# przemektmalon/SeqALib

Hardware: AMD Instinct MI355X
Metric: GCUPS (DP cell updates/s) on batched 4k×4k SW; bit-exact score match (higher is better)
Workload: dtype f16 (integer-exact below 2048); 1 GPU; sw_batch_10000x4096x4096; pairs_per_gpu=10000, total_pairs=10000, m=4096, n=4096, algo=SmithWatermanSA, match=equal<char>, parallelism=pair-shard x1

## Files before the change

### seqalib_amd/csrc/sa_api.hip

```cpp
#include <hip/hip_runtime.h>
#include <limits.h>
#include <sched.h>
#include <stdio.h>
#include <stdlib.h>
#include <string.h>

#include <algorithm>
#include <atomic>
#include <functional>
#include <condition_variable>
#include <memory>
#include <mutex>
#include <chrono>
#include <string>
#include <thread>
#include <vector>

#include "sa_dc.h"
#include "sa_internal.h"

using namespace sa;

namespace sa {
bool dna2_pack(uint8_t* dst, const uint8_t* src, uint64_t n);
// ... 459 lines not shown
        if (algo != SA_SW && algo != SA_NW && algo != SA_LOCAL_GOTOH && algo != SA_GLOBAL_GOTOH) return T16Mode{};
        const int64_t mi = is_affine(algo) ? 2 * ((int64_t)sc0->gap_open + sc0->gap_extend) - 1 : 2 * (int64_t)sc0->gap - 1;
        if (mi < INT_MIN / 4) return T16Mode{};
        eff.mismatch = (int32_t)mi;
        eff.allow_mismatch = 1;
    }
    const sa_scoring* sc = &eff;
    T16Mode t;
    t.mismatch = sc->mismatch;
    if (algo == SA_LOCAL_GOTOH || algo == SA_GLOBAL_GOTOH) return t16_mode_affine(algo, sc, max_m, max_n);
    if (algo != SA_SW && algo != SA_NW) return t;
    const int64_t MA = sc->match, MI = sc->mismatch, G = sc->gap;
    if (MA < -32 || MA > 31 || MI < -32 || MI > 31) return t;
    if (G > 0 || MI > MA || G < -4096) return t;
    if (algo == SA_SW && G == 0) return t;
    if (max_n >= 65535) return t;
    const int64_t m = max_m, n = max_n, k = std::min(m, n);
    if (algo == SA_SW) {
        t.ok = true;
        if (4 * std::max<int64_t>(MA, 0) * k + 3 > 32767) t.retry_above = (int32_t)(8191 - std::max<int64_t>(MA, 0));
        return t;
    }
    auto hi_at = [&](int64_t i, int64_t j) {
        return std::max(std::min(i, j) * MA + (i > j ? i - j : j - i) * G, (i + j) * G);
    };
    auto lo_at = [&](int64_t i, int64_t j) {
        return std::max(std::min(i, j) * MI + (i > j ? i - j : j - i) * G, (i + j) * G);
    };
    int64_t hi = INT64_MIN, lo = INT64_MAX;
    const int64_t pts[7][2] = {{0, 0}, {m, 0}, {0, n}, {k, k}, {m, n}, {k, n}, {m, k}};
    for (auto& q : pts) {
        hi = std::max(hi, hi_at(q[0], q[1]));
        lo = std::min(lo, lo_at(q[0], q[1]));
    }
    const int64_t cand_lo = lo + std::min<int64_t>(std::min(MI, G), 0);
    const int64_t delta = (hi + cand_lo) >> 1;
    if (4 * (hi - delta) + 3 > 32767 || 4 * (cand_lo - delta) < -32768) return t;
    t.ok = true;
    t.delta = (int32_t)delta;
    return t;
}

int validate_scoring(sa_ctx* c, int algo, const sa_scoring* s) {
    if (!s) return fail(c, SA_ERR_ARG, "scoring is NULL");
    if (algo < SA_SW || algo > SA_MYERS_MILLER) return fail(c, SA_ERR_ARG, "unknown algorithm");
    return SA_OK;
}

bool f16_hi_exact(int s) {
    if (s < -2048 || s > 2048) return false;
    const _Float16 h = (_Float16)(float)s;
    return (int)(float)h == s && (__builtin_bit_cast(uint16_t, h) & 0xffu) == 0;
}
bool so2_f16_scoring(const sa_ctx* c, int algo, const sa_scoring* sc, const T16Mode& tm) {
    if (algo != SA_SW || !tm.ok || c->f16_off) return false;
    if (const char* e = getenv("SEQALIB_SO2_F16")) if (e[0] == '0') return false;
    return f16_hi_exact(sc->match) && f16_hi_exact(tm.mismatch) && f16_hi_exact(-128);
}

T16Mode t16_candidate(int algo, const sa_scoring* sc, uint32_t max_m, uint32_t max_n, uint32_t npairs) {
    T16Mode t = t16_mode(algo, sc, max_m, max_n);
    if ((algo == SA_SW || algo == SA_LOCAL_GOTOH) && !keyed_ok(algo, sc, max_m, max_n)) t.ok = false;
    if (t.ok && algo == SA_GLOBAL_GOTOH && t.retry_above != INT_MAX &&
        make_variant(algo, max_m, max_n, npairs, true, true).pl.split)
        t.ok = false;
    if (const char* e16 = getenv("SEQALIB_T16")) if (e16[0] == '0') t.ok = false;
    return t;
}

int build_variants(int algo, uint32_t max_m, uint32_t max_n, uint32_t npairs, bool t16, Variant (&vars)[3],
                   bool* has_fb, int only = 0) {
    int nv = 0;
    if (t16 && only != 2) vars[nv++] = make_variant(algo, max_m, max_n, npairs, true, true);
    if (!t16 || only != 1) vars[nv++] = make_variant(algo, max_m, max_n, npairs, false, true);
    *has_fb = false;
    for (int k = 0; k < nv; ++k) *has_fb = *has_fb || vars[k].pl.split;
    if (*has_fb) vars[nv] = make_variant(algo, max_m, max_n, npairs, false, false);
    const int all = nv + (*has_fb ? 1 : 0);
    uint64_t dir_stride = 0;
    for (int k = 0; k < all; ++k) dir_stride = std::max(dir_stride, vars[k].pl.g.dir_slot);
    for (int k = 0; k < all; ++k) {
        vars[k].slot_bytes += dir_stride - vars[k].pl.g.dir_slot;
        vars[k].pl.g.dir_slot = dir_stride;
    }
    return nv;
}

struct HostAlphabet {
    int sel = -1;
    uint32_t prof[5] = {0, 0, 0, 0, 0};
};
HostAlphabet host_alphabet(const uint8_t* s1, uint64_t t1, const uint8_t* s2, uint64_t t2, const uint8_t* lut,
                           int match, int mismatch, bool affine) {
    HostAlphabet h;
    bool seen[256] = {};
    for (uint64_t k = 0; k < t1; ++k) seen[s1[k]] = true;
    for (uint64_t k = 0; k < t2; ++k) seen[s2[k]] = true;
    uint32_t syms[4] = {0, 0, 0, 0};
    int nsym = 0;
    for (int b = 0; b < 256; ++b)
        if (seen[b]) {
            if (nsym == 4) { h.sel = 0; return h; }
            syms[nsym++] = (uint32_t)b;
        }
    for (int b = 0; nsym < 4 && b < 256; ++b)
        if (!seen[b]) syms[nsym++] = (uint32_t)b;
    for (int c = 0; c < 4; ++c) {
        uint32_t w = 0;
        for (int c2 = 0; c2 < 4; ++c2) {
            const bool v = lut ? lut[syms[c] * 256 + syms[c2]] != 0 : syms[c] == syms[c2];
// ... 32 lines not shown
    const bool allow = sc->allow_mismatch != 0;
    const bool bits = d_mbits != nullptr;
    const bool lut = !bits && d_lutbits != nullptr;
    const T16Mode tm = bits ? T16Mode{} : t16_candidate(algo, sc, max_m, max_n, npairs);
    const bool t16 = tm.ok;
    const bool kernel_timing = getenv("SEQALIB_KERNEL_TIMING") != nullptr;
    if (!c->aux) SA_HIP(c, hipMalloc(&c->aux, kPipeSlots * kAuxWords * 4));
    if (!c->h_sel) {
        SA_HIP(c, hipHostMalloc(reinterpret_cast<void**>(&c->h_sel), 64, hipHostMallocDefault));
        SA_HIP(c, hipEventCreateWithFlags(&c->ev_sel, hipEventDisableTiming));
    }
    if (!pipe && c->s_fill) {
        SA_HIP(c, hipStreamSynchronize(c->s_fill));
        SA_HIP(c, hipStreamSynchronize(c->s_tb));
    }
    constexpr int nslots = kPipeSlots;
    const int slot = pipe ? (int)(c->pipe_k % (uint64_t)nslots) : 0;
    uint32_t* aux = c->aux + kAuxWords * slot;
    if (pipe && c->ev_slot[slot]) SA_HIP(c, hipStreamWaitEvent(stream, c->ev_slot[slot], 0));
    if (!c->h_f16) {
        SA_HIP(c, hipHostMalloc(reinterpret_cast<void**>(&c->h_f16), 8, hipHostMallocCoherent));
        *c->h_f16 = 0;
        void* dp = nullptr;
        SA_HIP(c, hipHostGetDevicePointer(&dp, c->h_f16, 0));
        c->d_f16 = static_cast<unsigned long long*>(dp);
    }
    {
        const unsigned long long w = __atomic_load_n(c->h_f16, __ATOMIC_ACQUIRE);
        const uint32_t s = (uint32_t)(w >> 32);
        if (s != 0 && s != c->f16_seen) {
            c->f16_seen = s;
            if (c->f16_seq - s < 4 && (uint64_t)(uint32_t)w * 64 > c->f16_cnt[s & 3]) c->f16_off = true;
        }
    }
    const uint32_t* sel = nullptr;
    const uint32_t* prof = aux + kAuxProf;
    static_assert(kAuxSel == kAuxProf + 5, "profile and selection word: one upload");
    int only = 0;
    HostAlphabet hal;
    if (t16 && hs) hal = host_alphabet(hs->s1, hs->t1, hs->s2, hs->t2, hs->lut, sc->match, tm.mismatch, is_affine(algo));
    const HostAlphabet* ha = &hal;
    const bool host_sel = t16 && ha->sel >= 0;
    if (host_sel) {
        c->host_sel = ha->sel;
        const bool in_hdr = hs->hhdr != nullptr;
        if (!in_hdr && !hs->hprof) return fail(c, SA_ERR_ARG, "internal: no pinned profile slot");
        uint32_t* const hp = in_hdr ? hs->hhdr : hs->hprof;
        for (int k = 0; k < 5; ++k) hp[k] = ha->prof[k];
        hp[5] = (uint32_t)ha->sel;
        if (in_hdr) prof = hs->dhdr;
        else SA_HIP(c, hipMemcpyAsync(aux + kAuxProf, hp, 24, hipMemcpyHostToDevice, stream));
        const Variant vt = make_variant(algo, max_m, max_n, npairs, true, true);
        const bool bu_hand = vt.so && !is_affine(algo) && (vt.pl.g.bands > 1 || vt.segs > 1);
        const bool f16 = vt.so2 && so2_f16_scoring(c, algo, sc, tm);
        if (ha->sel == 0) only = 2;
        else if (tm.retry_above == INT_MAX && !bu_hand && !f16) only = 1;
        else sel = prof + 5;
    }
    if (hs && hs->up_bytes)
        SA_HIP(c, hipMemcpyAsync(hs->up_dst, hs->up_src, hs->up_bytes, hipMemcpyHostToDevice, stream));
    if (host_sel) {
        SA_HIP(c, hipEventRecord(c->ev_sel, stream));
    } else if (t16) {
        c->host_sel = -1;
        SA_HIP(c, launch_alphabet_scan(d1, o1, d2, o2, npairs, aux, stream));
        SA_HIP(c, launch_decide_t16(d_lutbits, sc->match, tm.mismatch, is_affine(algo) ? 1 : 0, aux, stream));
        SA_HIP(c, hipMemcpyAsync(c->h_sel, aux + kAuxSel, 4, hipMemcpyDeviceToHost, stream));
        SA_HIP(c, hipEventRecord(c->ev_sel, stream));
        sel = aux + kAuxSel;
    }
    Variant vars[3];
    bool has_fb = false;
    const int nv = build_variants(algo, max_m, max_n, npairs, t16, vars, &has_fb, only);
    if (const char* e = getenv("SEQALIB_SPLIT_FALLBACK")) has_fb = has_fb && e[0] != '0';
    c->nvar = nv;
    uint64_t slot_bytes = 0, sp_bands = 0;
    bool any_split = false;
    for (int k = 0; k < nv + (has_fb ? 1 : 0); ++k) {
        if (k < nv) {
            c->var_kernel[k] = vars[k].kernel;
            c->var_R[k] = vars[k].pl.R;
            c->var_W[k] = vars[k].pl.split ? 0 : vars[k].pl.W;
            c->var_records[k] = vars[k].so ? SA_RECORDS_SCORE_ONLY : vars[k].t16 ? SA_RECORDS_TAGS : SA_RECORDS_FLAGS;
        }
        slot_bytes = std::max(slot_bytes, vars[k].slot_bytes);
        if (vars[k].pl.split) {
            any_split = true;
            sp_bands = std::max<uint64_t>(sp_bands, vars[k].pl.g.bands);
        }
    }
    const uint64_t budget = pipe ? ws_budget(c) / nslots : ws_budget(c);
    uint64_t per_launch = slot_bytes ? std::max<uint64_t>(1, budget / std::max<uint64_t>(slot_bytes, 1)) : npairs;
    per_launch = std::min<uint64_t>(per_launch, npairs ? npairs : 1);
    per_launch = std::min<uint64_t>(per_launch, 1u << 30);
    const uint64_t need = (per_launch * slot_bytes + 4096 + 255) & ~(uint64_t)255;
    if (need > budget && per_launch == 1 && c->ws_limit)
        return fail(c, SA_ERR_NOMEM, "one pair needs " + std::to_string(slot_bytes) +
                                         " bytes of workspace, above the limit");
    int rc = ensure_ws(c, std::max<uint64_t>(pipe ? nslots * need : need, 4096));
    if (rc) return rc;
    auto al256 = [](uint64_t x) { return (x + 255) & ~(uint64_t)255; };
    uint64_t hand_rb = 0, hand_part = 0, hand_seg = 0;
    for (int k = 0; k < nv; ++k)
        if (vars[k].so && !is_affine(algo)) {
            hand_rb = std::max(hand_rb, al256(per_launch * vars[k].pl.rowbuf_elems * 4));
            hand_part = std::max(hand_part, al256(per_launch * vars[k].part_slot * 8));
            hand_seg = std::max(hand_seg, al256(per_launch * vars[k].seg_slot * 4));
// ... 85 lines not shown
            fp.mbits = d_mbits; fp.mbits_off = d_mbits_off;
            fp.dirs = wbase; fp.dir_slot = pl.g.dir_slot; fp.band_stride = pl.g.band_stride;
            fp.rowbuf = rowbuf; fp.rowbuf_slot = pl.rowbuf_elems;
            fp.res = d_res;
            fp.pair_base = (uint32_t)base;
            fp.max_m = max_m; fp.max_n = max_n;
            fp.gap = sc->gap; fp.match = sc->match;
            fp.mismatch = v.t16 ? tm.mismatch : allow ? sc->mismatch : INT_MIN;
            fp.gap_open = sc->gap_open; fp.gap_extend = sc->gap_extend;
            fp.waves = pl.W;
            fp.count = cnt;
            fp.stage_seq2 = (max_n <= kMaxStagedSeq2 && !no_stage) ? 1 : 0;
            fp.prof = prof;
            const bool fb = k == nv;
            fp.sel = fb ? nullptr : sel; fp.sel_want = v.t16 ? 1u : 0u;
            fp.redo = (!fb && nv == 2 && !v.t16) ? 1 : 0;
            fp.rerun = fb ? 1 : 0;
            fp.t16_delta = v.t16 ? tm.delta : 0;
            fp.retry_above = v.t16 ? tm.retry_above : INT_MAX;
            fp.t16_sent = v.t16 ? tm.sent : -10000;
            fp.snap_h = snap_h; fp.snap_p = snap_p; fp.snap_m = snap_p + per_launch * v.snap_p_slot;
            if (v.so) {
                fp.part_bands = (uint32_t)v.pl.g.bands;
                fp.snap_c = reinterpret_cast<int32_t*>(snap_p + 2 * per_launch * v.snap_p_slot);
                fp.seg_slot = v.seg_slot;
            }
            if (v.so && !is_affine(algo)) {
                fp.epoch = c->hand_tag;
#ifndef SA_R5_CONTROL
                fp.rowbuf = reinterpret_cast<int32_t*>(c->hand);
                fp.band_part = reinterpret_cast<unsigned long long*>(c->hand + hand_rb);
                fp.seg_hand = reinterpret_cast<uint32_t*>(c->hand + hand_rb + hand_part);
#else
                const uintptr_t bp = (reinterpret_cast<uintptr_t>(fp.snap_c + per_launch * v.snap_c_slot) + 7) & ~(uintptr_t)7;
                fp.band_part = reinterpret_cast<unsigned long long*>(bp);
                fp.seg_hand = reinterpret_cast<uint32_t*>(fp.band_part + per_launch * v.part_slot);
#endif
                fp.wait_polls = so_wait_polls;
            }
            fp.snap_h_slot = v.snap_h_slot; fp.snap_p_slot = v.snap_p_slot; fp.snap_nch = v.snap_nch;
            fp.split_bands = (uint32_t)sp_bands;
            fp.ticket = pl.split ? reinterpret_cast<uint32_t*>(vblk) : v.so ? aux + kAuxTicket : nullptr;
            fp.hand = pl.split ? reinterpret_cast<unsigned long long*>(vblk + 256) : nullptr;
            fp.hand_x_off = pl.split ? hand_x_off : 0;
            fp.part = pl.split ? reinterpret_cast<int32_t*>(spbase + sp_part) : nullptr;
            fp.wait_ticks = wait_ticks;
            fp.part_segs = std::max<uint32_t>(1, v.segs);
            if (v.so2) {
                const uint32_t nch = chunks_per_band(max_n);
                const uint32_t sg = std::max(1u, std::min(fp.part_segs, nch / 2));
                const uint32_t range = std::max((nch + sg - 1) / sg, 3u) * kChunk + kWave;
                const uint32_t cap = (range + 15) & ~15u;
                fp.so2_stage = (2 * cap <= 8192 && !no_stage) ? cap : 0;
                if (v.t16 && so2_f16_scoring(c, algo, sc, tm)) {
                    fp.so2_f16 = 1;
                    fp.retry_above = std::min(fp.retry_above, kSo2F16RetryAbove);
                }
            }
            FillVariant fv{pl.R, lut, allow || v.t16, keyed, v.t16, v.cmax, pl.split, bits};
            fv.so = v.so;
            fv.so2 = v.so2;
            return fv;
        };
        const bool tb_on_fill = pipe && nv == 2 && !vars[1].t16 && !vars[1].pl.split;
        auto make_tp = [&](int k) {
            const Variant& v = vars[k];
            TbParams tp{};
            tp.seq1 = d1; tp.off1 = o1; tp.seq2 = d2; tp.off2 = o2;
            tp.lutbits = lut ? d_lutbits : nullptr;
            tp.vrec = bits ? 1 : 0;
            tp.dirs = fps[k].dirs; tp.dir_slot = v.pl.g.dir_slot;
            tp.ops = d_ops; tp.res = d_res;
            tp.pair_base = (uint32_t)base; tp.count = cnt;
            tp.max_m = max_m; tp.max_n = max_n;
            tp.gap = fps[k].gap; tp.match = fps[k].match; tp.mismatch = fps[k].mismatch;
            tp.gap_open = fps[k].gap_open; tp.gap_extend = fps[k].gap_extend;
            tp.allow = (allow || v.t16) ? 1 : 0;
            tp.tagged = v.t16 ? 1 : 0;
            tp.sel = fps[k].sel; tp.sel_want = fps[k].sel_want;
            tp.rerun = fps[k].rerun;
            tp.band_stride = v.pl.g.band_stride;
            tp.snap_h = fps[k].snap_h; tp.snap_p = fps[k].snap_p;
            tp.snap_h_slot = v.snap_h_slot; tp.snap_p_slot = v.snap_p_slot; tp.snap_nch = v.snap_nch;
            tp.prof = fps[k].prof;
            tp.t16_delta = fps[k].t16_delta;
            tp.t16_sent = fps[k].t16_sent;
            tp.so_lp = pipe ? 4 : 8;
            tp.keep_redo = tb_on_fill && k == 1 ? 1 : 0;
            tp.clear_redo = tb_on_fill && k == 0 ? 1 : 0;
#ifdef SA_R5_CONTROL
            tp.keep_redo = tp.clear_redo = 0;
#endif
            return tp;
        };
        for (int k = 0; k < nv; ++k) {
            const Variant& v = vars[k];
            const Plan& pl = v.pl;
            if (v.so && !is_affine(algo))
                if (int rc = next_hand_tag(c, hand_need, sf)) return rc;
            const FillVariant fv = make_fp(k);
            const FillParams& fp = fps[k];
            if (pl.split) SA_HIP(c, hipMemsetAsync(fp.ticket, 0, 256 + hand_x_off * 8 * aff2, sf));
            if (v.so && !is_affine(algo)) SA_HIP(c, hipMemsetAsync(fp.ticket, 0, 8, sf));
            static_assert(kAuxF16Flags == kAuxTicket + 1, "ticket and f16 count: one memset");
            if (kev) SA_HIP(c, hipEventRecord(kev[2 * k], sf));
            const bool units = v.so && !is_affine(algo);
            const uint32_t grid = pl.split ? (uint32_t)(cnt * sp_bands)
                                : units ? (v.so2 ? (cnt + 1) / 2 : cnt) * pl.g.bands * v.segs : cnt;
// ... 1086 lines not shown
```

### seqalib_amd/csrc/sa_fill_so2.hip

```cpp
#include "sa_fill_impl.h"

namespace sa {

namespace {

__device__ __forceinline__ uint32_t pk_max_u16(uint32_t a, uint32_t b) {
    uint32_t d;
    asm("v_pk_max_u16 %0, %1, %2" : "=v"(d) : "v"(a), "v"(b));
    return d;
}
__device__ __forceinline__ uint32_t lo16(uint32_t x) { return x & 0xffffu; }
__device__ __forceinline__ uint32_t lane_here() {
    uint32_t l;
    asm volatile("v_mov_b32 %0, %1" : "=v"(l) : "v"((uint32_t)threadIdx.x));
    return l;
}
__device__ __forceinline__ uint32_t hi16(uint32_t x) { return x >> 16; }
__device__ __forceinline__ uint32_t wave_pk_max(uint32_t v) {
    v = pk_max_u16(v, (uint32_t)__builtin_amdgcn_update_dpp(0, (int)v, 0x111, 0xf, 0xf, false));
    v = pk_max_u16(v, (uint32_t)__builtin_amdgcn_update_dpp(0, (int)v, 0x112, 0xf, 0xf, false));
    v = pk_max_u16(v, (uint32_t)__builtin_amdgcn_update_dpp(0, (int)v, 0x114, 0xf, 0xf, false));
    v = pk_max_u16(v, (uint32_t)__builtin_amdgcn_update_dpp(0, (int)v, 0x118, 0xf, 0xf, false));
    v = pk_max_u16(v, (uint32_t)__builtin_amdgcn_update_dpp(0, (int)v, 0x142, 0xa, 0xf, false));
    v = pk_max_u16(v, (uint32_t)__builtin_amdgcn_update_dpp(0, (int)v, 0x143, 0xc, 0xf, false));
    return v;
}
__device__ __forceinline__ uint32_t pk_max_i16(uint32_t a, uint32_t b) {
    uint32_t d;
    asm("v_pk_max_i16 %0, %1, %2" : "=v"(d) : "v"(a), "v"(b));
    return d;
}
__device__ __forceinline__ uint32_t f16x2_to_u16x2(uint32_t x) {
    uint32_t d;
    asm("v_cvt_u16_f16_sdwa %0, %1 dst_sel:WORD_0 dst_unused:UNUSED_PAD src0_sel:WORD_0\n\t"
        "v_cvt_u16_f16_sdwa %0, %1 dst_sel:WORD_1 dst_unused:UNUSED_PRESERVE src0_sel:WORD_1"
        : "=&v"(d) : "v"(x));
    return d;
}
__device__ __forceinline__ uint32_t u16x2_to_f16x2(uint32_t x) {
    uint32_t d;
    asm("v_cvt_f16_u16_sdwa %0, %1 dst_sel:WORD_0 dst_unused:UNUSED_PAD src0_sel:WORD_0\n\t"
        "v_cvt_f16_u16_sdwa %0, %1 dst_sel:WORD_1 dst_unused:UNUSED_PRESERVE src0_sel:WORD_1"
        : "=&v"(d) : "v"(x));
    return d;
}
__device__ __forceinline__ uint32_t f16_bits(int s) {
    const _Float16 h = (_Float16)(float)s;
    return (uint32_t)__builtin_bit_cast(uint16_t, h);
}

}

template <int ALG, int R, bool FK>
__global__ __launch_bounds__(64) __attribute__((amdgpu_waves_per_eu(4, 4))) void fill_so2_kernel(FillParams P) {
    constexpr bool NWK = ALG == SA_NW;
    static_assert(!(FK && NWK), "the f16 cell is SW's");
    if (sa_skip(P.sel, P.sel_want)) return;
    static_assert(R >= 8 && R % 2 == 0, "the sampled chunk maximum needs 8 rows per lane");
    constexpr int BAND = kWave * R;
    constexpr int SPP = 8;
    extern __shared__ __attribute__((aligned(16))) uint32_t smem[];
    uint32_t* const s_step = smem;
    const int lane = threadIdx.x;
    uint32_t* const s_park = s_step + (lane == 63 ? 96 : 160);
    const uint32_t SEGS = P.part_segs;
    const uint32_t ncp = (P.count + 1) / 2;
    uint32_t t = 0;
    if (lane == 0) t = atomicAdd(P.ticket, 1u);
    t = __builtin_amdgcn_readlane(t, 0);
    const uint32_t rowt = ncp * SEGS;
    const uint32_t band0 = t / rowt;
    const uint32_t rem = t - band0 * rowt;
    const uint32_t seg = rem / ncp;
    const uint32_t cp = rem - seg * ncp;
    const uint32_t sA = 2 * cp;
    const bool hasB = 2 * cp + 1 < P.count;
    const uint32_t sB = hasB ? 2 * cp + 1 : sA;
    const uint32_t pA = P.pair_base + sA, pB = P.pair_base + sB;
    const uint64_t o1A = P.off1[pA], o2A = P.off2[pA], o1B = P.off1[pB], o2B = P.off2[pB];
    const int mA = (int)(P.off1[pA + 1] - o1A), nA = (int)(P.off2[pA + 1] - o2A);
    const int mB = hasB ? (int)(P.off1[pB + 1] - o1B) : 0, nB = hasB ? (int)(P.off2[pB + 1] - o2B) : 0;
    const bool badA = (uint32_t)mA > P.max_m || (uint32_t)nA > P.max_n;
    const bool badB = hasB && ((uint32_t)mB > P.max_m || (uint32_t)nB > P.max_n);
    const int BA = (!badA && mA > 0 && nA > 0) ? (mA + BAND - 1) / BAND : 0;
    const int BB = (hasB && !badB && mB > 0 && nB > 0) ? (mB + BAND - 1) / BAND : 0;
    const int B2 = max(BA, BB);
    const int n2 = max(BA ? nA : 0, BB ? nB : 0);
    if ((int)band0 >= (B2 > 0 ? B2 : 1)) return;
    const uint32_t nch2 = chunks_per_band((uint32_t)n2);
    const uint32_t segs_p = max(1u, min(SEGS, nch2 / 2));
    const uint32_t cps = (nch2 + segs_p - 1) / segs_p;
    const uint32_t c0 = seg * cps, c1 = B2 > 0 ? min(nch2, c0 + cps) : 0u;
    const uint32_t last_seg = (nch2 - 1) / cps;
    if (seg > (B2 > 0 ? last_seg : 0u)) return;
    const uint32_t nchA = chunks_per_band((uint32_t)nA), nchB = chunks_per_band((uint32_t)nB);
    const bool liveA = (int)band0 < BA, liveB = (int)band0 < BB;
    const uint32_t epoch16 = P.epoch << 16;
    const uint32_t symp = P.prof[4];
    const int G = P.gap;
    const int D0 = P.t16_delta;
    auto border2 = [&](int i) __attribute__((always_inline)) -> uint32_t {
        return NWK ? ((uint32_t)(i * G - D0) & 0xffffu) * 0x10001u : 0u;
    };
    uint32_t seg_lost = 0;

    uint32_t cw[4];
#pragma unroll
    for (int c = 0; c < 4; ++c) {
        uint32_t w = 0;
#pragma unroll
        for (int x = 0; x < 4; ++x) {
            const int s = (int)(int8_t)(so_profile(P.prof[x]) >> (8 * c));
            if constexpr (FK) w |= (f16_bits(s) >> 8) << (8 * x);
            else w |= ((uint32_t)(s + 128) & 255u) << (8 * x);
        }
        cw[c] = w;
    }
    const uint8_t* const s1A = P.seq1 + o1A;
    const uint8_t* const s1B = P.seq1 + o1B;
    const uint8_t* const s2A = P.seq2 + o2A;
    const uint8_t* const s2B = P.seq2 + o2B;
    const bool staged = P.so2_stage != 0;
    const int k0 = max(0, (int)(c0 * kChunk) - kWave);
    uint8_t* const s_cA = reinterpret_cast<uint8_t*>(smem + kStepBufWords);
    uint8_t* const s_cB = s_cA + P.so2_stage;
    if (staged) {
        const int k1 = min(n2, (int)(c1 * kChunk));
        for (int k = k0 + lane; k < k1; k += kWave) {
            s_cA[k - k0] = (uint8_t)(liveA && k < nA ? t16_code8(symp, s2A[(uint32_t)k]) >> 3 : 0u);
            s_cB[k - k0] = (uint8_t)(liveB && k < nB ? t16_code8(symp, s2B[(uint32_t)k]) >> 3 : 0u);
        }
        __syncthreads();
    }
    constexpr uint32_t kOut = FK ? 0xd8d8d8d8u : 0u;
    auto col_pair = [&](int c, uint32_t& wa, uint32_t& wb) {
        const bool ia = liveA && c >= 0 && c < nA, ib = liveB && c >= 0 && c < nB;
        uint32_t xa, xb;
        if (staged) {
            xa = ia ? (uint32_t)s_cA[c - k0] : 0u;
            xb = ib ? (uint32_t)s_cB[c - k0] : 0u;
        } else {
            xa = ia ? (t16_code8(symp, s2A[(uint32_t)c]) >> 3) : 0u;
            xb = ib ? (t16_code8(symp, s2B[(uint32_t)c]) >> 3) : 0u;
        }
        wa = ia ? (xa == 0 ? cw[0] : xa == 1 ? cw[1] : xa == 2 ? cw[2] : cw[3]) : kOut;
        wb = ib ? (xb == 0 ? cw[0] : xb == 1 ? cw[1] : xb == 2 ? cw[2] : cw[3]) : kOut;
    };
    const uint32_t G128 = FK ? f16_bits(G) * 0x10001u : ((uint32_t)(G + 128) & 0xffffu) * 0x10001u;
    const uint32_t C128 = 0x00800080u;

    typedef uint32_t __attribute__((address_space(1))) gu32;
    gu32* const rbA = (gu32*)(P.rowbuf + (uint64_t)sA * P.rowbuf_slot);
    gu32* const rbB = (gu32*)(P.rowbuf + (uint64_t)sB * P.rowbuf_slot);
    const uint64_t rbs = P.max_n;

    const int row0 = (int)band0 * BAND + lane * R;
    uint32_t Hp[R], sel[R];
    uint32_t prev_up = border2(row0), colA = 0, colB = 0, cml = 0, smax = 0;
#pragma unroll
    for (int r = 0; r < R; ++r) Hp[r] = border2(row0 + r + 1);
    int capSA = -1, capSB = -1, capIA = 0, capIB = 0;
    uint32_t capA = 0, capB = 0;
    bool tookA = false, tookB = false;
    if constexpr (NWK) {
        if (liveA && mA > 0 && nA > 0 && (int)band0 == (mA - 1) / BAND) {
            capIA = (mA - 1) % BAND;
            capSA = nA - 1 + capIA / R;
        }
        if (liveB && mB > 0 && nB > 0 && (int)band0 == (mB - 1) / BAND) {
            capIB = (mB - 1) % BAND;
            capSB = nB - 1 + capIB / R;
        }
    }
    if (c0 > 0) {
        const uint64_t hoff = ((uint64_t)band0 * SEGS + seg - 1) * (R + 1) * kWave;
        const uint32_t* const hsA = P.seg_hand + (uint64_t)sA * P.seg_slot + hoff;
        const uint32_t* const hsB = P.seg_hand + (uint64_t)sB * P.seg_slot + hoff;
        uint32_t pa_ = 0, pb_ = 0;
        auto rd = [&]() __attribute__((always_inline)) {
#pragma unroll
            for (int r = 0; r < R; ++r) {
                Hp[r] = liveA ? __hip_atomic_load(hsA + (uint32_t)(r * kWave + lane), __ATOMIC_RELAXED, __HIP_MEMORY_SCOPE_AGENT) : epoch16;
                sel[r] = liveB ? __hip_atomic_load(hsB + (uint32_t)(r * kWave + lane), __ATOMIC_RELAXED, __HIP_MEMORY_SCOPE_AGENT) : epoch16;
            }
            pa_ = liveA ? __hip_atomic_load(hsA + (uint32_t)(R * kWave + lane), __ATOMIC_RELAXED, __HIP_MEMORY_SCOPE_AGENT) : epoch16;
            pb_ = liveB ? __hip_atomic_load(hsB + (uint32_t)(R * kWave + lane), __ATOMIC_RELAXED, __HIP_MEMORY_SCOPE_AGENT) : epoch16;
        };
        auto stale = [&]() __attribute__((always_inline)) -> bool {
            bool st = ((pa_ & 0xffff0000u) != epoch16) | ((pb_ & 0xffff0000u) != epoch16);
#pragma unroll
            for (int r = 0; r < R; ++r) st |= ((Hp[r] & 0xffff0000u) != epoch16) | ((sel[r] & 0xffff0000u) != epoch16);
            return st;
        };
        rd();
        for (uint32_t it = 0; !seg_lost && __builtin_amdgcn_ballot_w64(stale()) != 0; ++it) {
            if (it >= P.wait_polls) { seg_lost = 1; break; }
            __builtin_amdgcn_s_sleep(2);
            rd();
        }
#pragma unroll
        for (int r = 0; r < R; ++r) Hp[r] = lo16(Hp[r]) | sel[r] << 16;
        prev_up = lo16(pa_) | pb_ << 16;
        col_pair((int)(c0 * kChunk) - 1 - lane, colA, colB);
    }
#pragma unroll
    for (int r = 0; r < R; ++r) {
        const int row = row0 + r;
        const uint32_t ca = (liveA && row < mA) ? (t16_code8(symp, s1A[(uint32_t)row]) >> 3) : 12u;
        const uint32_t cb = (liveB && row < mB) ? (4u + (t16_code8(symp, s1B[(uint32_t)row]) >> 3)) : 12u;
        sel[r] = FK ? 0x0cu | ca << 8 | 0x0c0000u | cb << 24 : ca | 0x0c00u | cb << 16 | 0x0c000000u;
    }

    auto step = [&](auto ramp, auto gc, int kC, int q0, const uint32_t* sq, const uint32_t* sc, uint32_t* sp,
                    uint32_t& recA, uint32_t& recB) {
        constexpr bool RAMP = decltype(ramp)::value;
        constexpr int g = decltype(gc)::value;
        constexpr int PH = g & 3;
        const int q = q0 + g;
        const uint32_t vh = sq[g];
        const uint32_t va = sc[2 * g], vb = sc[2 * g + 1];
        const uint32_t up = (uint32_t)shr1((int)vh, (int)Hp[R - 1]);
        colA = (uint32_t)shr1((int)va, (int)colA);
        colB = (uint32_t)shr1((int)vb, (int)colB);
        if (!RAMP || kC + q - lane >= 0) {
            uint32_t dcur, pt;
            if constexpr (FK)
                asm("v_perm_b32 %1, %2, %3, %4\n\tv_pk_add_f16 %0, %5, %1"
                    : "=&v"(dcur), "=&v"(pt) : "v"(colB), "v"(colA), "v"(sel[0]), "v"(prev_up));
            else
                asm("v_perm_b32 %1, %2, %3, %4\n\tv_pk_add_u16 %0, %5, %1"
                    : "=&v"(dcur), "=&v"(pt) : "v"(colB), "v"(colA), "v"(sel[0]), "v"(prev_up));
            uint32_t hu = up;
#define SO2_CELL_N(LAST)                                                                          \
    asm("v_perm_b32 %[dn], %[cb], %[ca], %[sn]\n\t"                                                \
        "v_pk_add_u16 %[dn], %[hp], %[dn]\n\t"                                                     \
        "v_pk_max_i16 %[t1], %[hu], %[hp]\n\t"                                                     \
        "v_pk_add_u16 %[t1], %[t1], %[g]\n\t"                                                      \
        "v_pk_max_i16 %[t1], %[t1], %[dr]\n\t" LAST                                                \
        : [t1] "=&v"(t1), [dn] "=&v"(dn), [hp] "+v"(Hp[r])                                         \
        : [dr] "v"(dcur), [hu] "v"(hu), [g] "s"(G128), [c] "s"(C128),                              \
          [sn] "v"(sel[r + 1 < R ? r + 1 : r]), [ca] "v"(colA), [cb] "v"(colB))
#define SO2_CELL_L(LAST)                                                                          \
    asm("v_pk_max_i16 %[t1], %[hu], %[hp]\n\t"                                                     \
        "v_pk_add_u16 %[t1], %[t1], %[g]\n\t"                                                      \
        "v_pk_max_i16 %[t1], %[t1], %[dr]\n\t" LAST                                                \
        : [t1] "=&v"(t1), [hp] "+v"(Hp[r])                                                         \
        : [dr] "v"(dcur), [hu] "v"(hu), [g] "s"(G128), [c] "s"(C128))
#define SO2_CELL_FN                                                                               \
    asm("v_perm_b32 %[dn], %[cb], %[ca], %[sn]\n\t"                                                \
        "v_pk_add_f16 %[dn], %[hp], %[dn]\n\t"                                                     \
        "v_pk_max_i16 %[t1], %[hu], %[hp]\n\t"                                                     \
        "v_pk_add_f16 %[t1], %[t1], %[g]\n\t"                                                      \
        "v_pk_maximum3_f16 %[hp], %[t1], %[dr], 0"                                                 \
        : [t1] "=&v"(t1), [dn] "=&v"(dn), [hp] "+v"(Hp[r])                                         \
        : [dr] "v"(dcur), [hu] "v"(hu), [g] "s"(G128),                                             \
          [sn] "v"(sel[r + 1 < R ? r + 1 : r]), [ca] "v"(colA), [cb] "v"(colB))
#define SO2_CELL_FL                                                                               \
    asm("v_pk_max_i16 %[t1], %[hu], %[hp]\n\t"                                                     \
        "v_pk_add_f16 %[t1], %[t1], %[g]\n\t"                                                      \
        "v_pk_maximum3_f16 %[hp], %[t1], %[dr], 0"                                                 \
        : [t1] "=&v"(t1), [hp] "+v"(Hp[r])                                                         \
        : [dr] "v"(dcur), [hu] "v"(hu), [g] "s"(G128))
#pragma unroll
            for (int r = 0; r < R; ++r) {
                uint32_t t1;
                if (r + 1 < R) {
                    uint32_t dn;
                    if constexpr (FK) SO2_CELL_FN;
                    else if constexpr (NWK) SO2_CELL_N("v_pk_sub_u16 %[hp], %[t1], %[c]");
                    else SO2_CELL_N("v_pk_sub_u16 %[hp], %[t1], %[c] clamp");
                    dcur = dn;
                } else {
                    if constexpr (FK) SO2_CELL_FL;
                    else if constexpr (NWK) SO2_CELL_L("v_pk_sub_u16 %[hp], %[t1], %[c]");
                    else SO2_CELL_L("v_pk_sub_u16 %[hp], %[t1], %[c] clamp");
                }
                if (!NWK && PH == 3 && (r & 7) == 7) {
                    if constexpr (FK) {
                        cml = pk_max_i16(cml, Hp[r - 4]);
                        cml = pk_max_i16(cml, Hp[r]);
                    } else {
                        cml = pk_max_u16(cml, Hp[r - 4]);
                        cml = pk_max_u16(cml, Hp[r]);
                    }
                }
                hu = Hp[r];
            }
#undef SO2_CELL_N
#undef SO2_CELL_L
#undef SO2_CELL_FN
#undef SO2_CELL_FL
            prev_up = up;
        }
        if constexpr (NWK) {
            if (kC + q == capSA) {
                uint32_t v = 0;
#pragma unroll
                for (int r = 0; r < R; ++r) v = r == capIA % R ? Hp[r] : v;
                capA = lane == capIA / R ? lo16(v) : capA;
                tookA = true;
            }
            if (kC + q == capSB) {
                uint32_t v = 0;
#pragma unroll
                for (int r = 0; r < R; ++r) v = r == capIB % R ? Hp[r] : v;
                capB = lane == capIB / R ? hi16(v) : capB;
                tookB = true;
            }
        }
        recA = __builtin_amdgcn_alignbit(Hp[R - 1], recA, 16u);
        recB = __builtin_amdgcn_perm(Hp[R - 1], recB, 0x07060302u);
        sp[g] = Hp[R - 1];
    };

    uint8_t* const dA = P.dirs + (uint64_t)sA * P.dir_slot + (uint64_t)band0 * P.band_stride;
    uint8_t* const dB = P.dirs + (uint64_t)sB * P.dir_slot + (uint64_t)band0 * P.band_stride;
    gu32* const gA = rbA + (uint64_t)(band0 > 0 ? band0 - 1 : 0) * rbs;
    gu32* const gB = rbB + (uint64_t)(band0 > 0 ? band0 - 1 : 0) * rbs;
    gu32* const oA = rbA + (uint64_t)band0 * rbs;
    gu32* const oB = rbB + (uint64_t)band0 * rbs;
    for (uint32_t chunk = c0; chunk < c1; ++chunk) {
        const int kC = (int)chunk * kChunk;
        {
            const uint32_t ln = lane_here();
            const int c = kC + (int)ln;
            const bool in = lane < kChunk;
            uint32_t wa = 0, wb = 0;
            if (in) col_pair(c, wa, wb);
            const bool wantA = in && band0 > 0 && liveA && c < nA, wantB = in && band0 > 0 && liveB && c < nB;
            gu32* const ga = gA + (uint32_t)c;
            gu32* const gb = gB + (uint32_t)c;
            uint32_t ha = lo16(border2(c + 1)), hb = ha;
            if (wantA) ha = __hip_atomic_load(ga, __ATOMIC_RELAXED, __HIP_MEMORY_SCOPE_AGENT);
            if (wantB) hb = __hip_atomic_load(gb, __ATOMIC_RELAXED, __HIP_MEMORY_SCOPE_AGENT);
            if (band0 > 0) {
                for (uint32_t it = 0; !seg_lost; ++it) {
                    const bool st = (wantA && (ha & 0xffff0000u) != epoch16) || (wantB && (hb & 0xffff0000u) != epoch16);
                    if (__builtin_amdgcn_ballot_w64(st) == 0) break;
                    if (it >= P.wait_polls) { seg_lost = 1; break; }
                    __builtin_amdgcn_s_sleep(2);
                    if (wantA) ha = __hip_atomic_load(ga, __ATOMIC_RELAXED, __HIP_MEMORY_SCOPE_AGENT);
                    if (wantB) hb = __hip_atomic_load(gb, __ATOMIC_RELAXED, __HIP_MEMORY_SCOPE_AGENT);
                }
            }
            if (in) {
                s_step[ln] = FK ? u16x2_to_f16x2(lo16(ha) | hb << 16) : lo16(ha) | hb << 16;
                s_step[32 + 2 * ln] = wa;
                s_step[33 + 2 * ln] = wb;
            }
        }
        __syncthreads();
        auto packet = [&](auto rmp, int q0) __attribute__((always_inline)) {
            uint32_t pa[SPP / 2] = {0, 0, 0, 0}, pb[SPP / 2] = {0, 0, 0, 0};
            const uint32_t* const sq = s_step + q0;
            const uint32_t* const sc = s_step + 32 + 2 * q0;
            uint32_t* const sp = s_park + q0;
            auto st = [&](auto gc) __attribute__((always_inline)) {
                constexpr int g = decltype(gc)::value;
                step(rmp, gc, kC, q0, sq, sc, sp, pa[g / 2], pb[g / 2]);
            };
            st(std::integral_constant<int, 0>{});
            st(std::integral_constant<int, 1>{});
            st(std::integral_constant<int, 2>{});
            st(std::integral_constant<int, 3>{});
            st(std::integral_constant<int, 4>{});
            st(std::integral_constant<int, 5>{});
            st(std::integral_constant<int, 6>{});
            st(std::integral_constant<int, 7>{});
            const uint32_t po = ((uint32_t)((kC + q0) / SPP) * kWave + (uint32_t)lane) * 16u;
            if constexpr (FK) {
#pragma unroll
                for (int w = 0; w < SPP / 2; ++w) {
                    pa[w] = f16x2_to_u16x2(pa[w]);
                    pb[w] = f16x2_to_u16x2(pb[w]);
                }
            }
            if (liveA) {
                const u32x4 v4 = {pa[0], pa[1], pa[2], pa[3]};
                __builtin_nontemporal_store(v4, reinterpret_cast<u32x4*>(dA + po));
            }
            if (liveB) {
                const u32x4 v4 = {pb[0], pb[1], pb[2], pb[3]};
                __builtin_nontemporal_store(v4, reinterpret_cast<u32x4*>(dB + po));
            }
        };
        if (kC < kWave - 1) {
#pragma unroll 1
            for (int q0 = 0; q0 < kChunk; q0 += SPP) packet(std::true_type{}, q0);
        } else {
#pragma unroll 1
            for (int q0 = 0; q0 < kChunk; q0 += SPP) packet(std::false_type{}, q0);
        }
        const uint32_t ln = lane_here();
        {
            uint32_t acc = s_step[96 + (ln & 31)];
            if constexpr (FK) acc = f16x2_to_u16x2(acc);
            const int cc = kC + (int)ln - (kWave - 1);
            if (lane < kChunk && cc >= 0) {
                if ((int)band0 + 1 < BA && cc < nA)
                    __hip_atomic_store(oA + (uint32_t)cc, epoch16 | lo16(acc), __ATOMIC_RELAXED, __HIP_MEMORY_SCOPE_AGENT);
                if ((int)band0 + 1 < BB && cc < nB)
                    __hip_atomic_store(oB + (uint32_t)cc, epoch16 | hi16(acc), __ATOMIC_RELAXED, __HIP_MEMORY_SCOPE_AGENT);
            }
        }
        {
            const uint64_t e = (uint64_t)band0 * P.snap_nch + chunk;
            if (kC + kChunk - 1 < lane) cml = 0;
            if constexpr (FK) cml = f16x2_to_u16x2(cml);
            smax = pk_max_u16(smax, cml);
            const uint32_t wm = NWK ? 0u : wave_pk_max(cml);
            const uint32_t pup = FK ? f16x2_to_u16x2(prev_up) : prev_up;
            if (liveA && chunk < nchA) {
                if constexpr (!NWK) {
                    int32_t* const smA = P.snap_m + (uint64_t)sA * P.snap_p_slot + e * kWave;
                    smA[ln] = (int32_t)lo16(cml);
                    if (lane == kWave - 1) P.snap_c[(uint64_t)sA * P.part_bands * P.snap_nch + e] = (int32_t)lo16(wm);
                }
                if (chunk + 1 < nchA) {
                    uint32_t* const sh = P.snap_h + (uint64_t)sA * P.snap_h_slot + e * (R / 2) * kWave + ln;
#pragma unroll
                    for (int q = 0; q < R / 2; ++q) {
                        const uint32_t w = __builtin_amdgcn_perm(Hp[2 * q + 1], Hp[2 * q], 0x05040100u);
                        sh[q * kWave] = FK ? f16x2_to_u16x2(w) : w;
                    }
                    int32_t* const spA = P.snap_p + (uint64_t)sA * P.snap_p_slot + e * kWave;
                    spA[ln] = (int32_t)lo16(pup);
                }
            }
            if (liveB && chunk < nchB) {
                if constexpr (!NWK) {
                    int32_t* const smB = P.snap_m + (uint64_t)sB * P.snap_p_slot + e * kWave;
                    smB[ln] = (int32_t)hi16(cml);
                    if (lane == kWave - 1) P.snap_c[(uint64_t)sB * P.part_bands * P.snap_nch + e] = (int32_t)hi16(wm);
                }
                if (chunk + 1 < nchB) {
                    uint32_t* const sh = P.snap_h + (uint64_t)sB * P.snap_h_slot + e * (R / 2) * kWave + ln;
#pragma unroll
                    for (int q = 0; q < R / 2; ++q) {
                        const uint32_t w = __builtin_amdgcn_perm(Hp[2 * q + 1], Hp[2 * q], 0x07060302u);
                        sh[q * kWave] = FK ? f16x2_to_u16x2(w) : w;
                    }
                    int32_t* const spB = P.snap_p + (uint64_t)sB * P.snap_p_slot + e * kWave;
                    spB[ln] = (int32_t)hi16(pup);
                }
            }
            cml = 0;
        }
        if (chunk + 1 == c1 && c1 < nch2) {
            const uint64_t hoff = ((uint64_t)band0 * SEGS + seg) * (R + 1) * kWave;
            if (liveA) {
                uint32_t* const hs = P.seg_hand + (uint64_t)sA * P.seg_slot + hoff + ln;
#pragma unroll
                for (int r = 0; r < R; ++r)
                    __hip_atomic_store(hs + r * kWave, epoch16 | lo16(Hp[r]), __ATOMIC_RELAXED, __HIP_MEMORY_SCOPE_AGENT);
                __hip_atomic_store(hs + R * kWave, epoch16 | lo16(prev_up), __ATOMIC_RELAXED, __HIP_MEMORY_SCOPE_AGENT);
            }
            if (liveB) {
                uint32_t* const hs = P.seg_hand + (uint64_t)sB * P.seg_slot + hoff + ln;
#pragma unroll
                for (int r = 0; r < R; ++r)
                    __hip_atomic_store(hs + r * kWave, epoch16 | hi16(Hp[r]), __ATOMIC_RELAXED, __HIP_MEMORY_SCOPE_AGENT);
                __hip_atomic_store(hs + R * kWave, epoch16 | hi16(prev_up), __ATOMIC_RELAXED, __HIP_MEMORY_SCOPE_AGENT);
            }
        }
        __syncthreads();
    }

    seg_lost = __builtin_amdgcn_ballot_w64(seg_lost != 0) != 0 ? 1u : 0u;
    uint32_t wA = 0, wB = 0;
    if constexpr (NWK) {
        if (tookA) wA = 1u << 16 | (((uint32_t)__builtin_amdgcn_readlane((int)capA, capIA / R) & 0xffffu) ^ 0x8000u);
        if (tookB) wB = 1u << 16 | (((uint32_t)__builtin_amdgcn_readlane((int)capB, capIB / R) & 0xffffu) ^ 0x8000u);
    } else {
#pragma unroll
        for (int off = 32; off >= 1; off >>= 1) smax = pk_max_u16(smax, (uint32_t)__shfl_xor((int)smax, off));
        wA = liveA ? lo16(smax) : 0u;
        wB = liveB ? hi16(smax) : 0u;
    }
    typedef unsigned long long __attribute__((address_space(1))) gu64p;
    gu64p* const partA = (gu64p*)(P.band_part + (uint64_t)sA * P.part_bands * SEGS);
    gu64p* const partB = (gu64p*)(P.band_part + (uint64_t)sB * P.part_bands * SEGS);
    const uint32_t me = band0 * SEGS + seg, nparts = B2 > 0 ? (uint32_t)(B2 - 1) * SEGS + last_seg : 0u;
    if (me != nparts) {
        if (lane == 0) {
            __hip_atomic_store(partA + me, (unsigned long long)epoch16 << 32 | wA | seg_lost << 31,
                               __ATOMIC_RELAXED, __HIP_MEMORY_SCOPE_AGENT);
            if (hasB)
                __hip_atomic_store(partB + me, (unsigned long long)epoch16 << 32 | wB | seg_lost << 31,
                                   __ATOMIC_RELAXED, __HIP_MEMORY_SCOPE_AGENT);
        }
        return;
    }
    uint32_t lostA = seg_lost, lostB = seg_lost;
    uint32_t mxA = bu_fold_parts(partA, nparts, last_seg, SEGS, epoch16, P.wait_polls, lane, lostA);
    uint32_t mxB = hasB ? bu_fold_parts(partB, nparts, last_seg, SEGS, epoch16, P.wait_polls, lane, lostB) : 0u;
    mxA = max(mxA, wA);
    mxB = max(mxB, wB);
#pragma unroll
    for (int off = 32; off >= 1; off >>= 1) {
        mxA = max(mxA, (uint32_t)__shfl_xor((int)mxA, off));
        mxB = max(mxB, (uint32_t)__shfl_xor((int)mxB, off));
    }
    if (lane == 0) {
        auto report = [&](uint32_t pidx, bool bad, int Bx, int mx_, int nx_, uint32_t mx, uint32_t lost) {
            sa_result r = {};
            if (bad) {
                r.flags = SA_FLAG_BAD_SHAPE;
            } else if constexpr (NWK) {
                r.end_i = mx_;
                r.end_j = nx_;
                if (Bx == 0) {
                    r.score = (mx_ > nx_ ? mx_ : nx_) * G;
                } else {
                    r.score = (int)(int16_t)(uint16_t)((mx & 0xffffu) ^ 0x8000u) + D0;
                    if (!((mx >> 16) & 1u) || lost) r.flags |= kFlagRetry;
                }
            } else if (Bx == 0) {
                r.score = INT_MIN;
            } else {
                r.score = (int)mx;
                r.reserved = 1;
                if ((int)mx - kSoSlack * G > P.retry_above) {
                    r.flags |= kFlagRetry;
                    if constexpr (FK) atomicAdd(P.ticket + (kAuxF16Flags - kAuxTicket), 1u);
                }
                if (lost) r.flags |= kFlagRetry;
            }
            P.res[pidx] = r;
        };
        report(pA, badA, BA, mA, nA, mxA, lostA);
        if (hasB) report(pB, badB, BB, mB, nB, mxB, lostB);
    }
}

hipError_t launch_fill_so2(int algo, int R, const FillParams& p, uint32_t grid, hipStream_t stream) {
    const size_t lds = (size_t)kStepBufWords * 4 + 2 * (size_t)p.so2_stage;
#define SO2_LAUNCH(A, RR, F)                                                                        \
    if (algo == (A) && R == (RR) && (p.so2_f16 != 0) == (F)) {                                      \
        hipLaunchKernelGGL((fill_so2_kernel<A, RR, F>), dim3(grid), dim3(kWave), lds, stream, p);  \
        return hipGetLastError();                                                                  \
    }
    SO2_LAUNCH(SA_SW, 32, true)
    SO2_LAUNCH(SA_SW, 16, true)
    SO2_LAUNCH(SA_SW, 32, false)
    SO2_LAUNCH(SA_SW, 16, false)
    SO2_LAUNCH(SA_NW, 32, false)
    SO2_LAUNCH(SA_NW, 16, false)
#undef SO2_LAUNCH
    return hipErrorInvalidValue;
}

}
```

Before: 11780 GCUPS.

## Add scaled-f16 SW cell variant carrying the gap-added up value per row

```diff
diff --git a/seqalib_amd/csrc/sa_api.hip b/seqalib_amd/csrc/sa_api.hip
--- a/seqalib_amd/csrc/sa_api.hip
+++ b/seqalib_amd/csrc/sa_api.hip
@@ -535,10 +535,14 @@
     const _Float16 h = (_Float16)(float)s;
     return (int)(float)h == s && (__builtin_bit_cast(uint16_t, h) & 0xffu) == 0;
 }
-bool so2_f16_scoring(const sa_ctx* c, int algo, const sa_scoring* sc, const T16Mode& tm) {
-    if (algo != SA_SW || !tm.ok || c->f16_off) return false;
-    if (const char* e = getenv("SEQALIB_SO2_F16")) if (e[0] == '0') return false;
-    return f16_hi_exact(sc->match) && f16_hi_exact(tm.mismatch) && f16_hi_exact(-128);
+uint32_t so2_f16_scoring(const sa_ctx* c, int algo, const sa_scoring* sc, const T16Mode& tm) {
+    if (algo != SA_SW || !tm.ok || c->f16_off) return 0;
+    uint32_t cell = 2;
+    if (const char* e = getenv("SEQALIB_SO2_F16")) {
+        if (e[0] == '0') return 0;
+        if (e[0] == '5') cell = 1;
+    }
+    return f16_hi_exact(sc->match) && f16_hi_exact(tm.mismatch) && f16_hi_exact(-128) ? cell : 0;
 }
 
 T16Mode t16_candidate(int algo, const sa_scoring* sc, uint32_t max_m, uint32_t max_n, uint32_t npairs) {
@@ -677,7 +681,7 @@
         else SA_HIP(c, hipMemcpyAsync(aux + kAuxProf, hp, 24, hipMemcpyHostToDevice, stream));
         const Variant vt = make_variant(algo, max_m, max_n, npairs, true, true);
         const bool bu_hand = vt.so && !is_affine(algo) && (vt.pl.g.bands > 1 || vt.segs > 1);
-        const bool f16 = vt.so2 && so2_f16_scoring(c, algo, sc, tm);
+        const bool f16 = vt.so2 && so2_f16_scoring(c, algo, sc, tm) != 0;
         if (ha->sel == 0) only = 2;
         else if (tm.retry_above == INT_MAX && !bu_hand && !f16) only = 1;
         else sel = prof + 5;
@@ -869,8 +873,8 @@
                 const uint32_t range = std::max((nch + sg - 1) / sg, 3u) * kChunk + kWave;
                 const uint32_t cap = (range + 15) & ~15u;
                 fp.so2_stage = (2 * cap <= 8192 && !no_stage) ? cap : 0;
-                if (v.t16 && so2_f16_scoring(c, algo, sc, tm)) {
-                    fp.so2_f16 = 1;
+                if (const uint32_t cell = v.t16 ? so2_f16_scoring(c, algo, sc, tm) : 0u) {
+                    fp.so2_f16 = cell;
                     fp.retry_above = std::min(fp.retry_above, kSo2F16RetryAbove);
                 }
             }
diff --git a/seqalib_amd/csrc/sa_fill_so2.hip b/seqalib_amd/csrc/sa_fill_so2.hip
--- a/seqalib_amd/csrc/sa_fill_so2.hip
+++ b/seqalib_amd/csrc/sa_fill_so2.hip
@@ -33,14 +33,18 @@
 __device__ __forceinline__ uint32_t f16x2_to_u16x2(uint32_t x) {
     uint32_t d;
     asm("v_cvt_u16_f16_sdwa %0, %1 dst_sel:WORD_0 dst_unused:UNUSED_PAD src0_sel:WORD_0\n\t"
-        "v_cvt_u16_f16_sdwa %0, %1 dst_sel:WORD_1 dst_unused:UNUSED_PRESERVE src0_sel:WORD_1"
+        "s_nop 0\n\t"
+        "v_cvt_u16_f16_sdwa %0, %1 dst_sel:WORD_1 dst_unused:UNUSED_PRESERVE src0_sel:WORD_1\n\t"
+        "s_nop 0"
         : "=&v"(d) : "v"(x));
     return d;
 }
 __device__ __forceinline__ uint32_t u16x2_to_f16x2(uint32_t x) {
     uint32_t d;
     asm("v_cvt_f16_u16_sdwa %0, %1 dst_sel:WORD_0 dst_unused:UNUSED_PAD src0_sel:WORD_0\n\t"
-        "v_cvt_f16_u16_sdwa %0, %1 dst_sel:WORD_1 dst_unused:UNUSED_PRESERVE src0_sel:WORD_1"
+        "s_nop 0\n\t"
+        "v_cvt_f16_u16_sdwa %0, %1 dst_sel:WORD_1 dst_unused:UNUSED_PRESERVE src0_sel:WORD_1\n\t"
+        "s_nop 0"
         : "=&v"(d) : "v"(x));
     return d;
 }
@@ -48,12 +52,39 @@
     const _Float16 h = (_Float16)(float)s;
     return (uint32_t)__builtin_bit_cast(uint16_t, h);
 }
-
-}
-
-template <int ALG, int R, bool FK>
-__global__ __launch_bounds__(64) __attribute__((amdgpu_waves_per_eu(4, 4))) void fill_so2_kernel(FillParams P) {
+__device__ __forceinline__ uint32_t f16_bits_sc(int s) {
+    const _Float16 h = (_Float16)((float)s * (1.0f / 2048.0f));
+    return (uint32_t)__builtin_bit_cast(uint16_t, h);
+}
+typedef _Float16 so2_h2 __attribute__((ext_vector_type(2)));
+__device__ __forceinline__ uint32_t sc_to_u16x2(uint32_t x) {
+    const so2_h2 k = {(_Float16)0.0001220703125f, (_Float16)0.0001220703125f};
+    return __builtin_bit_cast(uint32_t, __builtin_bit_cast(so2_h2, x) * k);
+}
+__device__ __forceinline__ uint32_t u16x2_to_sc(uint32_t x) {
+    const so2_h2 k = {(_Float16)8192.0f, (_Float16)8192.0f};
+    return __builtin_bit_cast(uint32_t, __builtin_bit_cast(so2_h2, x) * k);
+}
+__device__ __forceinline__ uint32_t pk_addg_clamp(uint32_t h, uint32_t g) {
+    uint32_t d;
+    asm("v_pk_add_f16 %0, %1, %2 clamp" : "=v"(d) : "v"(h), "s"(g));
+    return d;
+}
+template <int FK>
+__device__ __forceinline__ uint32_t so2_out(uint32_t x) {
+    if constexpr (FK == 2) return sc_to_u16x2(x);
+    else if constexpr (FK == 1) return f16x2_to_u16x2(x);
+    else return x;
+}
+constexpr int so2_waves(int FK, int R) { return FK == 2 && R == 32 ? 3 : 4; }
+
+}
+
+template <int ALG, int R, int FK>
+__global__ __launch_bounds__(64) __attribute__((amdgpu_waves_per_eu(so2_waves(FK, R), so2_waves(FK, R))))
+void fill_so2_kernel(FillParams P) {
     constexpr bool NWK = ALG == SA_NW;
+    constexpr bool X4 = FK == 2;
     static_assert(!(FK && NWK), "the f16 cell is SW's");
     if (sa_skip(P.sel, P.sel_want)) return;
     static_assert(R >= 8 && R % 2 == 0, "the sampled chunk maximum needs 8 rows per lane");
@@ -111,7 +142,8 @@
 #pragma unroll
         for (int x = 0; x < 4; ++x) {
             const int s = (int)(int8_t)(so_profile(P.prof[x]) >> (8 * c));
-            if constexpr (FK) w |= (f16_bits(s) >> 8) << (8 * x);
+            if constexpr (X4) w |= (f16_bits_sc(s) >> 8) << (8 * x);
+            else if constexpr (FK) w |= (f16_bits(s) >> 8) << (8 * x);
             else w |= ((uint32_t)(s + 128) & 255u) << (8 * x);
         }
         cw[c] = w;
@@ -132,7 +164,7 @@
         }
         __syncthreads();
     }
-    constexpr uint32_t kOut = FK ? 0xd8d8d8d8u : 0u;
+    constexpr uint32_t kOut = X4 ? 0xacacacacu : FK ? 0xd8d8d8d8u : 0u;
     auto col_pair = [&](int c, uint32_t& wa, uint32_t& wb) {
         const bool ia = liveA && c >= 0 && c < nA, ib = liveB && c >= 0 && c < nB;
         uint32_t xa, xb;
@@ -146,7 +178,9 @@
         wa = ia ? (xa == 0 ? cw[0] : xa == 1 ? cw[1] : xa == 2 ? cw[2] : cw[3]) : kOut;
         wb = ib ? (xb == 0 ? cw[0] : xb == 1 ? cw[1] : xb == 2 ? cw[2] : cw[3]) : kOut;
     };
-    const uint32_t G128 = FK ? f16_bits(G) * 0x10001u : ((uint32_t)(G + 128) & 0xffffu) * 0x10001u;
+    const uint32_t G128 = X4   ? f16_bits_sc(G) * 0x10001u
+                          : FK ? f16_bits(G) * 0x10001u
+                               : ((uint32_t)(G + 128) & 0xffffu) * 0x10001u;
     const uint32_t C128 = 0x00800080u;
 
     typedef uint32_t __attribute__((address_space(1))) gu32;
@@ -156,9 +190,12 @@
 
     const int row0 = (int)band0 * BAND + lane * R;
     uint32_t Hp[R], sel[R];
+    uint32_t Fr[X4 ? R : 1];
     uint32_t prev_up = border2(row0), colA = 0, colB = 0, cml = 0, smax = 0;
 #pragma unroll
     for (int r = 0; r < R; ++r) Hp[r] = border2(row0 + r + 1);
+#pragma unroll
+    for (int r = 0; r < (X4 ? R : 1); ++r) Fr[r] = 0;
     int capSA = -1, capSB = -1, capIA = 0, capIB = 0;
     uint32_t capA = 0, capB = 0;
     bool tookA = false, tookB = false;
@@ -200,6 +237,10 @@
         }
 #pragma unroll
         for (int r = 0; r < R; ++r) Hp[r] = lo16(Hp[r]) | sel[r] << 16;
+        if constexpr (X4) {
+#pragma unroll
+            for (int r = 0; r < R; ++r) Fr[r] = pk_addg_clamp(Hp[r], G128);
+        }
         prev_up = lo16(pa_) | pb_ << 16;
         col_pair((int)(c0 * kChunk) - 1 - lane, colA, colB);
     }
@@ -230,7 +271,7 @@
             else
                 asm("v_perm_b32 %1, %2, %3, %4\n\tv_pk_add_u16 %0, %5, %1"
                     : "=&v"(dcur), "=&v"(pt) : "v"(colB), "v"(colA), "v"(sel[0]), "v"(prev_up));
-            uint32_t hu = up;
+            uint32_t hu = X4 ? pk_addg_clamp(up, G128) : up;
 #define SO2_CELL_N(LAST)                                                                          \
     asm("v_perm_b32 %[dn], %[cb], %[ca], %[sn]\n\t"                                                \
         "v_pk_add_u16 %[dn], %[hp], %[dn]\n\t"                                                     \
@@ -261,17 +302,32 @@
         "v_pk_maximum3_f16 %[hp], %[t1], %[dr], 0"                                                 \
         : [t1] "=&v"(t1), [hp] "+v"(Hp[r])                                                         \
         : [dr] "v"(dcur), [hu] "v"(hu), [g] "s"(G128))
+#define SO2_CELL_XN                                                                               \
+    asm("v_perm_b32 %[dn], %[cb], %[ca], %[sn]\n\t"                                                \
+        "v_pk_add_f16 %[dn], %[hp], %[dn]\n\t"                                                     \
+        "v_pk_maximum3_f16 %[hp], %[dr], %[fu], %[fl]\n\t"                                         \
+        "v_pk_add_f16 %[fl], %[hp], %[g] clamp"                                                    \
+        : [dn] "=&v"(dn), [hp] "+v"(Hp[r]), [fl] "+v"(Fr[X4 ? r : 0])                              \
+        : [dr] "v"(dcur), [fu] "v"(hu), [g] "s"(G128),                                             \
+          [sn] "v"(sel[r + 1 < R ? r + 1 : r]), [ca] "v"(colA), [cb] "v"(colB))
+#define SO2_CELL_XL                                                                               \
+    asm("v_pk_maximum3_f16 %[hp], %[dr], %[fu], %[fl]\n\t"                                         \
+        "v_pk_add_f16 %[fl], %[hp], %[g] clamp"                                                    \
+        : [hp] "+v"(Hp[r]), [fl] "+v"(Fr[X4 ? r : 0])                                              \
+        : [dr] "v"(dcur), [fu] "v"(hu), [g] "s"(G128))
 #pragma unroll
             for (int r = 0; r < R; ++r) {
-                uint32_t t1;
+                [[maybe_unused]] uint32_t t1;
                 if (r + 1 < R) {
                     uint32_t dn;
-                    if constexpr (FK) SO2_CELL_FN;
+                    if constexpr (X4) SO2_CELL_XN;
+                    else if constexpr (FK) SO2_CELL_FN;
                     else if constexpr (NWK) SO2_CELL_N("v_pk_sub_u16 %[hp], %[t1], %[c]");
                     else SO2_CELL_N("v_pk_sub_u16 %[hp], %[t1], %[c] clamp");
                     dcur = dn;
                 } else {
-                    if constexpr (FK) SO2_CELL_FL;
+                    if constexpr (X4) SO2_CELL_XL;
+                    else if constexpr (FK) SO2_CELL_FL;
                     else if constexpr (NWK) SO2_CELL_L("v_pk_sub_u16 %[hp], %[t1], %[c]");
                     else SO2_CELL_L("v_pk_sub_u16 %[hp], %[t1], %[c] clamp");
                 }
@@ -284,8 +340,10 @@
                         cml = pk_max_u16(cml, Hp[r]);
                     }
                 }
-                hu = Hp[r];
-            }
+                hu = X4 ? Fr[X4 ? r : 0] : Hp[r];
+            }
+#undef SO2_CELL_XN
+#undef SO2_CELL_XL
 #undef SO2_CELL_N
 #undef SO2_CELL_L
 #undef SO2_CELL_FN
@@ -344,7 +402,8 @@
                 }
             }
             if (in) {
-                s_step[ln] = FK ? u16x2_to_f16x2(lo16(ha) | hb << 16) : lo16(ha) | hb << 16;
+                const uint32_t hab = lo16(ha) | hb << 16;
+                s_step[ln] = X4 ? u16x2_to_sc(hab) : FK ? u16x2_to_f16x2(hab) : hab;
                 s_step[32 + 2 * ln] = wa;
                 s_step[33 + 2 * ln] = wb;
             }
@@ -368,11 +427,11 @@
             st(std::integral_constant<int, 6>{});
             st(std::integral_constant<int, 7>{});
             const uint32_t po = ((uint32_t)((kC + q0) / SPP) * kWave + (uint32_t)lane) * 16u;
-            if constexpr (FK) {
+            if constexpr (FK != 0) {
 #pragma unroll
                 for (int w = 0; w < SPP / 2; ++w) {
-                    pa[w] = f16x2_to_u16x2(pa[w]);
-                    pb[w] = f16x2_to_u16x2(pb[w]);
+                    pa[w] = so2_out<FK>(pa[w]);
+                    pb[w] = so2_out<FK>(pb[w]);
                 }
             }
             if (liveA) {
@@ -384,7 +443,7 @@
                 __builtin_nontemporal_store(v4, reinterpret_cast<u32x4*>(dB + po));
             }
         };
-        if (kC < kWave - 1) {
+        if (!X4 && kC < kWave - 1) {
 #pragma unroll 1
             for (int q0 = 0; q0 < kChunk; q0 += SPP) packet(std::true_type{}, q0);
         } else {
@@ -394,7 +453,7 @@
         const uint32_t ln = lane_here();
         {
             uint32_t acc = s_step[96 + (ln & 31)];
-            if constexpr (FK) acc = f16x2_to_u16x2(acc);
+            acc = so2_out<FK>(acc);
             const int cc = kC + (int)ln - (kWave - 1);
             if (lane < kChunk && cc >= 0) {
                 if ((int)band0 + 1 < BA && cc < nA)
@@ -406,10 +465,10 @@
         {
             const uint64_t e = (uint64_t)band0 * P.snap_nch + chunk;
             if (kC + kChunk - 1 < lane) cml = 0;
-            if constexpr (FK) cml = f16x2_to_u16x2(cml);
+            cml = so2_out<FK>(cml);
             smax = pk_max_u16(smax, cml);
             const uint32_t wm = NWK ? 0u : wave_pk_max(cml);
-            const uint32_t pup = FK ? f16x2_to_u16x2(prev_up) : prev_up;
+            const uint32_t pup = so2_out<FK>(prev_up);
             if (liveA && chunk < nchA) {
                 if constexpr (!NWK) {
                     int32_t* const smA = P.snap_m + (uint64_t)sA * P.snap_p_slot + e * kWave;
@@ -421,7 +480,7 @@
 #pragma unroll
                     for (int q = 0; q < R / 2; ++q) {
                         const uint32_t w = __builtin_amdgcn_perm(Hp[2 * q + 1], Hp[2 * q], 0x05040100u);
-                        sh[q * kWave] = FK ? f16x2_to_u16x2(w) : w;
+                        sh[q * kWave] = so2_out<FK>(w);
                     }
                     int32_t* const spA = P.snap_p + (uint64_t)sA * P.snap_p_slot + e * kWave;
                     spA[ln] = (int32_t)lo16(pup);
@@ -438,7 +497,7 @@
 #pragma unroll
                     for (int q = 0; q < R / 2; ++q) {
                         const uint32_t w = __builtin_amdgcn_perm(Hp[2 * q + 1], Hp[2 * q], 0x07060302u);
-                        sh[q * kWave] = FK ? f16x2_to_u16x2(w) : w;
+                        sh[q * kWave] = so2_out<FK>(w);
                     }
                     int32_t* const spB = P.snap_p + (uint64_t)sB * P.snap_p_slot + e * kWave;
                     spB[ln] = (int32_t)hi16(pup);
@@ -536,16 +595,18 @@
 hipError_t launch_fill_so2(int algo, int R, const FillParams& p, uint32_t grid, hipStream_t stream) {
     const size_t lds = (size_t)kStepBufWords * 4 + 2 * (size_t)p.so2_stage;
 #define SO2_LAUNCH(A, RR, F)                                                                        \
-    if (algo == (A) && R == (RR) && (p.so2_f16 != 0) == (F)) {                                      \
+    if (algo == (A) && R == (RR) && (int)p.so2_f16 == (F)) {                                        \
         hipLaunchKernelGGL((fill_so2_kernel<A, RR, F>), dim3(grid), dim3(kWave), lds, stream, p);  \
         return hipGetLastError();                                                                  \
     }
-    SO2_LAUNCH(SA_SW, 32, true)
-    SO2_LAUNCH(SA_SW, 16, true)
-    SO2_LAUNCH(SA_SW, 32, false)
-    SO2_LAUNCH(SA_SW, 16, false)
-    SO2_LAUNCH(SA_NW, 32, false)
-    SO2_LAUNCH(SA_NW, 16, false)
+    SO2_LAUNCH(SA_SW, 32, 2)
+    SO2_LAUNCH(SA_SW, 16, 2)
+    SO2_LAUNCH(SA_SW, 32, 1)
+    SO2_LAUNCH(SA_SW, 16, 1)
+    SO2_LAUNCH(SA_SW, 32, 0)
+    SO2_LAUNCH(SA_SW, 16, 0)
+    SO2_LAUNCH(SA_NW, 32, 0)
+    SO2_LAUNCH(SA_NW, 16, 0)
 #undef SO2_LAUNCH
     return hipErrorInvalidValue;
 }
```

After: 13800 GCUPS, median of 6. 17.1% higher.
